# mhaseebtariq/doppel-speller

Hardware: AMD Instinct MI355X
Metric: candidate-pairs scored/sec (Jaccard top-k + Levenshtein), 100k x 500k titles (higher is better)
Workload: dtype f32 accumulate / f64 finalise (Jaccard), u8 + f64 ratio (Levenshtein)

## Files before the change

### doppel-speller_amd/csrc/ds_common.h

```cpp
#pragma once

#include <hip/hip_runtime.h>

#include <cstdarg>
#include <cstdint>
#include <cstdio>
#include <cstring>
#include <string>
#include <vector>

#include "doppel_amd.h"

namespace ds {

constexpr int kWideTileRows = 28672, kNarrowTileRows = 12288;
constexpr int64_t kNarrowMaxTruth = 5000000;
constexpr int kDenseThreads = 1024;
constexpr int kMaxQueryColumns = 128;
constexpr int kSignatureBits = 128;
constexpr int kSignatureWords = kSignatureBits / 32;
constexpr int kRowRecordWords = 8;
constexpr int kControlWords = 32;

inline uint32_t encode_sums8(float x)
{
    if (!(x >= 0.125f)) return 0u;
    uint32_t bits;
    memcpy(&bits, &x, sizeof(bits));
    const int exponent = static_cast<int>(bits >> 23) - 124;
    if (exponent > 15) return 0xfeu;
    return std::min<uint32_t>(0xfeu, (static_cast<uint32_t>(exponent) << 4) | ((bits >> 19) & 0xfu));
}

inline uint64_t mix64(uint64_t x)
{
    x ^= x >> 30;
    x *= 0xbf58476d1ce4e5b9ull;
    x ^= x >> 27;
    x *= 0x94d049bb133111ebull;
    x ^= x >> 31;
    return x;
}

enum QueryStatus : int32_t { kQueryDone = 0, kQuerySlow = 1, kQueryErrorTopN = 2, kQueryErrorArg = 3, kQueryErrorTies = 4, kQuerySlowFew = 5 };

void set_error(const char *format, ...);
void duplicate_ranks(const int64_t *rowptr, const int32_t *truth_idx, const float *sums32, int64_t V, int64_t N,
                     uint16_t *rank_out);
int hip_failed(hipError_t error, const char *what, const char *file, int line);

#define DS_HIP(call)                                                          \
    do {                                                                      \
        hipError_t ds_hip_error_ = (call);                                    \
        if (ds_hip_error_ != hipSuccess) return ::ds::hip_failed(ds_hip_error_, #call, __FILE__, __LINE__); \
    } while (0)

#define DS_REQUIRE(condition, ...)            \
    do {                                      \
        if (!(condition)) {                   \
            ::ds::set_error(__VA_ARGS__);     \
            return DS_E_ARG;                  \
        }                                     \
    } while (0)

template <typename T>
struct DeviceBuffer {
    T *ptr = nullptr;
    size_t count = 0;
    int allocate(size_t n)
    {
        release();
        if (n == 0) return DS_OK;
        DS_HIP(hipMalloc(reinterpret_cast<void **>(&ptr), n * sizeof(T)));
        count = n;
        return DS_OK;
    }
    int upload(const T *host, size_t n)
    {
        int status = allocate(n);
        if (status != DS_OK) return status;
        if (n) DS_HIP(hipMemcpy(ptr, host, n * sizeof(T), hipMemcpyHostToDevice));
        return DS_OK;
    }
    void release()
    {
// ... 68 lines not shown
```

### doppel-speller_amd/csrc/ds_jaccard_impl.inc

```
#include <cfloat>
#include <type_traits>
#include <cstdlib>

#include "ds_common.h"

namespace ds {
namespace DS_GEOMETRY_NAME {

constexpr int kTile = DS_TILE_ROWS;
constexpr uint32_t kPadWord = kTile / 2;
constexpr uint32_t kPadQuad = kPadWord * 0x10001u;
__device__ __forceinline__ uint32_t posting_row(uint32_t posting) { return ((posting & 0x7fffu) << 1) | (posting >> 15); }
constexpr int kThreads = DS_THREADS;
constexpr int kWorkgroupsPerCu = DS_WGS_PER_CU;
static_assert(kTile % 4096 == 0 && kTile < 65536, "tile rows: whole scan iterations, 15-bit word indexes");
static_assert(kThreads >= 256 && kThreads % 64 == 0, "the radix histogram is cleared by threads 0..255");
constexpr int kCandidates = DS_CANDIDATES;
constexpr int kSelectSlack = 128;
constexpr int kPtrTiles = DS_PTR_TILES;

struct JaccardArgs {
    const uint32_t *col_ptr;
    const uint16_t *postings;
    const uint16_t *posting_sums;
// ... 5 lines not shown
    const int8_t *sig_column;
    const void *row_start;
    const void *row_cols;
    int32_t forward_wide_start, forward_wide_cols;
    const int64_t *q_rowptr;
    const int32_t *q_cols;
    const double *q_maxint;
    int32_t *out_rows;
    int32_t *status;
    int32_t *control;
    int32_t *slow_list;
    const int32_t *take_order;
    unsigned long long *phase;
    int64_t n_truth;
    int64_t n_columns;
    int64_t n_queries;
    int32_t n_tiles;
    int32_t k;
    int32_t sparse_quads;
    int32_t literal_only;
    int32_t rows_sorted;
    int32_t select_min;
    int32_t select_growth;
    int64_t n_quads;
    int64_t nnz;
    float sums_min;
};

enum { kCtlQueue = 0, kCtlSlowCount = 1, kCtlErrors = 2, kCtlExact = 3, kCtlSelects = 4, kCtlSlowQueue = 5,
       kCtlSparseTiles = 6, kCtlDenseTiles = 7, kCtlSkippedColumns = 8, kCtlReason = 9 ,
       kCtlRedos = 15 ,
       kCtlRefines = 16, kCtlRawEntries = 17, kCtlSurvivors = 18, kCtlRawSparse = 19,
       kCtlBytes = 28  };

constexpr int kEpochTiles = DS_EPOCH_TILES;
static_assert(kEpochTiles >= 1 && kEpochTiles <= 256 && (kEpochTiles & (kEpochTiles - 1)) == 0, "epoch: a power of two, at most 256 tiles");
constexpr bool kEpochInBytes = static_cast<long long>(kTile + 2) * kEpochTiles > 65536;
constexpr int kEpochShift = kEpochInBytes ? 16 : 14;
static_assert(kEpochInBytes || kTile + 2 <= (1 << kEpochShift), "a local row (or a padding row, kTile + 1) and the epoch bits share 16 bits");
constexpr int kScoreWords = kTile / 2 + 16;
constexpr int kOffLo = kScoreWords * 4;
constexpr int kOffRow = kOffLo + kCandidates * 4;
constexpr int kOffRaw = kOffRow + kCandidates * 4;
constexpr int kOffRawTile = kOffRaw + (kThreads / 64) * 64 * 4;
constexpr int kOffCols = kOffRawTile + (kEpochInBytes ? (kThreads / 64) * 64 : 0);
constexpr int kOffIdf = kOffCols + kMaxQueryColumns * 4;
constexpr int kOffMass = kOffIdf + kMaxQueryColumns * 4;
constexpr int kOffBitIdf = kOffMass + kMaxQueryColumns * 4;
constexpr int kOffFixed = kOffBitIdf + kSignatureBits * 4;
constexpr int kOffRank = kOffFixed + kMaxQueryColumns * 4;
constexpr int kOffOrder = kOffRank + kMaxQueryColumns;
constexpr int kOffSigBit = kOffOrder + kMaxQueryColumns;
constexpr int kOffMassTable = kOffSigBit + kMaxQueryColumns;
constexpr int kOffPtr = kOffMassTable + 256 * 6;
constexpr int kOffHist = kOffMassTable;
constexpr int kOffQuadPrefix = kOffPtr + kMaxQueryColumns * (kPtrTiles + 1) * 4;
constexpr int kOffQuadBase = kOffQuadPrefix + kMaxQueryColumns * 4;
constexpr int kDirItems = 64, kDirColumns = 64;
constexpr int kOffDirEntry = kOffQuadBase + kMaxQueryColumns * 4;
constexpr int kOffDirMask = kOffDirEntry + 2 * kDirColumns * 8;
constexpr int kOffDirCount = kOffDirMask + 2 * kDirItems * 8;
constexpr int kOffCtrl = kOffDirCount + 2 * kDirItems;
constexpr int kFastLdsBytes = kOffCtrl + 192;
static_assert((kFastLdsBytes + 256) * kWorkgroupsPerCu <= 160 * 1024, "LDS budget of one CU exceeded");
constexpr int kExactRows = kCandidates * 24 + kMaxQueryColumns * 5 + kThreads * 2 <= kTile * 2 ? kCandidates : ((kTile * 2 - kMaxQueryColumns * 5 - kThreads * 2) / 24) & ~7;
constexpr int kExactValueOffset = kExactRows * 16;
constexpr int kExactSortedOffset = kExactValueOffset + kExactRows * 8;
constexpr int kExactCountOffset = kExactSortedOffset + kMaxQueryColumns * 5;
static_assert(kExactValueOffset % 8 == 0 && kExactCountOffset % 4 == 0 && kExactCountOffset + kThreads * 2 <= kTile * 2,
              "exact-stage scratch fits the tile");
static_assert(kMaxQueryColumns == 128, "two ballots cover the query's columns");
constexpr int kKeep = (kCandidates + kThreads - 1) / kThreads;
constexpr int kSelectTrigger = kCandidates - kSelectSlack;
constexpr int kWaves = kThreads / 64;
constexpr float kFixedOne = 65000.f;
constexpr int kProbeMaxK = kThreads / 4;
static_assert(2 * kThreads <= kCandidates - kSelectSlack, "two samples per thread fit the candidate buffer");

enum { kLQuery = 0, kLCount, kLOverflow, kLDigit, kLRemain, kLCoef, kLPre, kLCut, kLKth0, kLKth1, kLBad, kLItems,
       kLUnused12 , kLNonEssential, kLMass, kLSparse, kLSigMask , kLQuant = kLSigMask + 4 , kLEnd,
       kLStartTile = 29 ,
       kLFloor = 37 ,
       kLAhead = 38 ,
       kLTileMask = 32 , kLTileSkip = 36 ,
       kLStats = 24 ,
       kLBytes = 30  };
static_assert(kLEnd <= kLStats && kLStats + 5 <= kLBytes && kLBytes + 2 <= 32 && kLBytes % 2 == 0, "LDS control words");
static_assert(kLTileSkip < kLFloor && kLFloor < kLAhead && kLAhead + 2 <= 48, "LDS control words 32..47");

__device__ __forceinline__ int uniform(int v) { return __builtin_amdgcn_readfirstlane(v); }
__device__ __forceinline__ uint32_t uniform(uint32_t v) { return static_cast<uint32_t>(__builtin_amdgcn_readfirstlane(static_cast<int>(v))); }
__device__ __forceinline__ float uniform(float v) { return __int_as_float(__builtin_amdgcn_readfirstlane(__float_as_int(v))); }
__device__ __forceinline__ bool uniform(bool v) { return __builtin_amdgcn_readfirstlane(v ? 1 : 0) != 0; }

__device__ __forceinline__ float round_down_positive(double x)
{
    float f = static_cast<float>(x);
    if (static_cast<double>(f) > x) f = __uint_as_float(__float_as_uint(f) - 1u);
    return f;
}

__device__ __forceinline__ float round_up_positive(double x)
{
    float f = static_cast<float>(x);
    if (static_cast<double>(f) < x) f = __uint_as_float(__float_as_uint(f) + 1u);
    return f;
}
// ... 49 lines not shown
            const uint32_t key = keys[i];
            if ((key & mask) == prefix) atomicAdd(&hist[(key >> shift) & 255u], 1u);
        }
        __syncthreads();
        if (tid < 64) {
            const int b0 = 255 - 4 * lane;
            const uint32_t c0 = hist[b0], c1 = hist[b0 - 1], c2 = hist[b0 - 2], c3 = hist[b0 - 3];
            const uint32_t local = c0 + c1 + c2 + c3;
            const uint32_t inclusive = wave_inclusive_scan(local, lane);
            const uint32_t exclusive = inclusive - local;
            const uint32_t want = static_cast<uint32_t>(remaining);
            if (want > exclusive && want <= inclusive) {
                uint32_t r = want - exclusive;
                int digit = b0;
                if (r > c0) { r -= c0; digit = b0 - 1;
                    if (r > c1) { r -= c1; digit = b0 - 2;
                        if (r > c2) { r -= c2; digit = b0 - 3; } } }
                ctrl[kLDigit] = digit;
                ctrl[kLRemain] = static_cast<int32_t>(r);
            }
        }
        __syncthreads();
        prefix |= static_cast<uint32_t>(uniform(static_cast<int>(ctrl[kLDigit]))) << shift;
        mask |= 255u << shift;
        remaining = uniform(static_cast<int>(ctrl[kLRemain]));
    }
    return prefix;
}

struct Bounds {
    float coef;
    float pre;
    float mass;
    float maxint32;
};

__device__ __forceinline__ uint32_t max_of_packed8(uint4 v)
{
    typedef unsigned short packed2 __attribute__((ext_vector_type(2)));
    const packed2 a = __builtin_elementwise_max(__builtin_bit_cast(packed2, v.x), __builtin_bit_cast(packed2, v.y));
    const packed2 b = __builtin_elementwise_max(__builtin_bit_cast(packed2, v.z), __builtin_bit_cast(packed2, v.w));
    const uint32_t m = __builtin_bit_cast(uint32_t, __builtin_elementwise_max(a, b));
    return max(m & 0xffffu, m >> 16);
}

__device__ __forceinline__ uint32_t max_of_packed4(const uint32_t (&v)[4])
{
    typedef unsigned short packed2 __attribute__((ext_vector_type(2)));
    const packed2 a = __builtin_elementwise_max(__builtin_bit_cast(packed2, v[0]), __builtin_bit_cast(packed2, v[1]));
    const packed2 b = __builtin_elementwise_max(__builtin_bit_cast(packed2, v[2]), __builtin_bit_cast(packed2, v[3]));
    return __builtin_bit_cast(uint32_t, __builtin_elementwise_max(a, b));
}

__device__ __forceinline__ float decode_sums8(uint32_t code)
{
    return code == 0u ? 0.f : __uint_as_float((((code >> 4) + 124u) << 23) | ((code & 0xfu) << 19));
}

__device__ __forceinline__ bool may_qualify(float s, float sums, const Bounds &b)
{
    return s + b.mass >= b.coef * (sums + b.maxint32);
}

__device__ __forceinline__ bool candidate_key(float s, float sums, const Bounds &b, uint32_t &key)
{
    if (!(s >= b.coef * (sums + b.maxint32))) return false;
    const float denominator = sums + (b.maxint32 - s);
    const float approx = s / denominator;
    key = (denominator > 0.f && approx == approx) ? __float_as_uint(approx) : 0x7f800000u;
    return true;
}

struct Skipped {
    int count;
    uint32_t sig_mask[kSignatureWords];
};

__device__ __forceinline__ float complete_score(float s, uint4 signature, const Skipped &skipped, const float *bit_idf)
{
    const uint32_t words[kSignatureWords] = {signature.x, signature.y, signature.z, signature.w};
#pragma unroll
    for (int w = 0; w < kSignatureWords; ++w) {
        uint32_t bits = words[w] & skipped.sig_mask[w];
        while (bits) {
            s += bit_idf[w * 32 + __ffs(bits) - 1];
            bits &= bits - 1u;
        }
    }
    return s;
}


__device__ __forceinline__ void append_candidate(bool pass, uint32_t key, int32_t row, uint32_t *cand_key,
                                                 int32_t *cand_row, ControlWords ctrl, int lane)
{
    const unsigned long long votes = __ballot(pass);
    if (votes == 0) return;
    const int leader = __ffsll(votes) - 1;
    int base = 0;
    if (lane == leader) base = atomicAdd(ctrl.at(kLCount), __popcll(votes));
    base = __shfl(base, leader);
    if (pass) {
        const int slot = base + __popcll(votes & ((1ull << lane) - 1ull));
        if (slot < kCandidates) {
            cand_key[slot] = key;
            cand_row[slot] = row;
        } else {
            ctrl[kLOverflow] = 1;
        }
    }
}
// ... 8 lines not shown
    }
}
__device__ __forceinline__ bool in_bounds(int32_t *control, int site, int64_t index, int64_t limit)
{
    if (index >= 0 && index < limit) return true;
    record_violation(control, site, index, limit);
    return false;
}
#define DS_OK_INDEX(site, index, limit) in_bounds(a.control, site, static_cast<int64_t>(index), static_cast<int64_t>(limit))
#else
#define DS_OK_INDEX(site, index, limit) true
#endif

#ifdef DS_DIAGNOSTICS
#define DS_STAMP(slot)                                                     \
    do {                                                                   \
        if (a.phase != nullptr && tid == 0) {                              \
            const unsigned long long now_ = __builtin_amdgcn_s_memtime();  \
            phase_lds[slot] += now_ - stamp_;                              \
            stamp_ = now_;                                                 \
        }                                                                  \
    } while (0)
#define DS_COUNT(slot, value)                                              \
    do {                                                                   \
        if (a.phase != nullptr && tid == 0) atomicAdd(&a.control[slot], value); \
    } while (0)
#else
#define DS_STAMP(slot) do { } while (0)
#define DS_COUNT(slot, value) do { } while (0)
#endif

template <bool kCountBytes, bool kSecondSample>
__global__ __launch_bounds__(kThreads, kWorkgroupsPerCu * kThreads / 256) void ds_jaccard_topk_kernel(const void *arguments)
{
    const __attribute__((address_space(4))) JaccardArgs &a =
        *reinterpret_cast<const __attribute__((address_space(4))) JaccardArgs *>(reinterpret_cast<uintptr_t>(arguments));
#ifdef DS_DIAGNOSTICS
    unsigned long long stamp_ = a.phase != nullptr ? __builtin_amdgcn_s_memtime() : 0ull;
    __shared__ unsigned long long phase_lds[16];
    if (threadIdx.x < 16) phase_lds[threadIdx.x] = 0ull;
#endif
    extern __shared__ __align__(16) unsigned char lds[];
    uint32_t *cand_key = reinterpret_cast<uint32_t *>(lds + kOffLo);
    int32_t *cand_row = reinterpret_cast<int32_t *>(lds + kOffRow);
    int32_t *cols = reinterpret_cast<int32_t *>(lds + kOffCols);
    float *idf = reinterpret_cast<float *>(lds + kOffIdf);
    uint8_t *rank = reinterpret_cast<uint8_t *>(lds + kOffRank);
    uint8_t *order = reinterpret_cast<uint8_t *>(lds + kOffOrder);
    float *mass_upto = reinterpret_cast<float *>(lds + kOffMass);
    int8_t *sig_bit = reinterpret_cast<int8_t *>(lds + kOffSigBit);
    float *bit_idf = reinterpret_cast<float *>(lds + kOffBitIdf);
    uint32_t *fixed = reinterpret_cast<uint32_t *>(lds + kOffFixed);
    uint32_t *iscores = reinterpret_cast<uint32_t *>(lds);
    uint32_t *need32 = reinterpret_cast<uint32_t *>(lds + kOffMassTable);
    uint16_t *mass16 = reinterpret_cast<uint16_t *>(lds + kOffMassTable + 256 * 4);
    uint32_t *ptr_cache = reinterpret_cast<uint32_t *>(lds + kOffPtr);
    uint32_t *quad_prefix = reinterpret_cast<uint32_t *>(lds + kOffQuadPrefix);
    uint32_t *quad_base = reinterpret_cast<uint32_t *>(lds + kOffQuadBase);
    uint2 *dir_entry = reinterpret_cast<uint2 *>(lds + kOffDirEntry);
    uint32_t *dir_mask = reinterpret_cast<uint32_t *>(lds + kOffDirMask);
    uint8_t *dir_count = reinterpret_cast<uint8_t *>(lds + kOffDirCount);
    uint32_t *hist = reinterpret_cast<uint32_t *>(lds + kOffHist);
    const ControlWords ctrl{reinterpret_cast<int32_t *>(lds + kOffCtrl)};

    const int tid = threadIdx.x, lane = tid & 63;
    const int wave = uniform(tid >> 6);
    const int k = a.k;
    const int64_t ptr_stride = static_cast<int64_t>(a.n_tiles) + 1;
    typedef const unsigned long long __attribute__((address_space(1))) *GlobalQuads;
    auto load_quad = [](GlobalQuads base, uint32_t at) {
        const unsigned long long bits = base[at];
        return make_uint2(static_cast<uint32_t>(bits), static_cast<uint32_t>(bits >> 32));
    };
    auto own_registers = [](const void *pointer) {
        const uint64_t bits = reinterpret_cast<uint64_t>(pointer);
        const uint32_t lo = uniform(static_cast<uint32_t>(bits)), hi = uniform(static_cast<uint32_t>(bits >> 32));
        return reinterpret_cast<GlobalQuads>((static_cast<uint64_t>(hi) << 32) | lo);
    };
    const GlobalQuads quads = own_registers(a.postings), sums_quads = own_registers(a.posting_sums);
    typedef const float __attribute__((address_space(4))) *ConstantFloats;
    const ConstantFloats tile_sums_min = reinterpret_cast<ConstantFloats>(reinterpret_cast<uintptr_t>(a.tile_sums_min));
    const ConstantFloats tile_sums_max = reinterpret_cast<ConstantFloats>(reinterpret_cast<uintptr_t>(a.tile_sums_max));

    for (int i = tid * 4; i < kScoreWords; i += kThreads * 4)
        *reinterpret_cast<uint4 *>(&iscores[i]) = make_uint4(0u, 0u, 0u, 0u);
    if (tid < 5) ctrl[kLStats + tid] = 0;
    if (tid < 2) ctrl[kLBytes + tid] = 0;
    __syncthreads();
    unsigned long long *requested = reinterpret_cast<unsigned long long *>(lds + kOffCtrl + kLBytes * 4);
    uint32_t query_units = 0;
    auto count_units = [&](uint32_t units) { if constexpr (kCountBytes) query_units += units; };

    for (;;) {
        if (tid == 0) {
            ctrl[kLQuery] = atomicAdd(&a.control[kCtlQueue], 1);
            ctrl[kLCount] = 0;
            ctrl[kLOverflow] = 0;
            ctrl[kLBad] = 0;
            ctrl[kLQuant] = 0;
            ctrl[kLStartTile] = 0;
            ctrl[kLFloor] = 0;
        }
        __syncthreads();
        const int64_t position = uniform(static_cast<int>(ctrl[kLQuery]));
        if (position >= a.n_queries) break;
        const int64_t q = a.take_order != nullptr ? static_cast<int64_t>(a.take_order[position]) : position;

        const int64_t qbase = a.q_rowptr[q];
// ... 156 lines not shown
            }
            raw_count += count;
        };

        int sparse_retries = 0;
        uint32_t dir_copy = 0;
        constexpr int kRound = 3;
        bool ahead = false;
        uint2 quad[kRound], quad_info[kRound];
        uint32_t quad_value[kRound];
        bool live[kRound];
#pragma unroll
        for (int u = 0; u < kRound; ++u) {
            quad[u] = quad_info[u] = make_uint2(0u, 0u);
            quad_value[u] = 0u;
            live[u] = false;
        }
        const int span = n > 0 ? min(a.n_tiles, max(kPtrTiles, kMaxQueryColumns * (kPtrTiles + 1) / n - 1)) : kPtrTiles;
        int block_start = 0, block_end = 0;
        const bool sorted = a.rows_sorted != 0;
        const int start_tile = sorted ? min(uniform(static_cast<int>(ctrl[kLStartTile])), a.n_tiles - 1) : 0;
        int epoch_start = start_tile, epoch_last = start_tile;
        int down_next = start_tile - 1;
        int up_next = start_tile + 1;
        bool descending = false;
        int run_left = 0;
        int b = start_tile;
        while (!slow) {
            bool redo_tile = false;
            const float tile_min = tile_sums_min[b];
            if (__builtin_expect(b < block_start || b >= block_end, 0)) {
                block_start = descending ? max(0, min(b, epoch_last - span + 1)) : b;
                block_end = block_start + span;
                __syncthreads();
                const int width = min(span, a.n_tiles - block_start) + 1;
                for (int e = tid; e < n * (span + 1); e += kThreads) {
                    const int j = e / (span + 1), i = e - j * (span + 1);
                    ptr_cache[e] = (i < width && DS_OK_INDEX(2, static_cast<int64_t>(cols[j]) * ptr_stride + block_start + i,
                                                            a.n_columns * ptr_stride))
                                       ? a.col_ptr[static_cast<int64_t>(cols[j]) * ptr_stride + block_start + i]
                                       : 0u;
                }
                count_units(static_cast<uint32_t>(n * width + 1) >> 1);
                __syncthreads();
            }
            const int bt = b - block_start;
            bounds.mass = pending_mass;
            if (__builtin_expect(rebuild_mass_table, 0)) {
                rebuild_mass_table = false;
                tables_fresh = true;
                if (tid < 4) ctrl[kLTileMask + tid] = static_cast<int32_t>(ctrl[kLSigMask + tid]);
                if (tid == 4) ctrl[kLTileSkip] = non_essential;
                if (tid < 256) {
                    const uint32_t skipped8 = static_cast<uint32_t>(ctrl[kLSigMask]) & 0xffu;
                    float rest = bounds.mass, some = 0.f;
                    for (int g = 0; g < 8; ++g) {
                        if (!((skipped8 >> g) & 1u)) continue;
                        rest -= bit_idf[g];
                        if ((tid >> g) & 1) some += bit_idf[g];
                    }
                    if (rest < 0.f) rest = 0.f;
                    const float value = (rest + some) * (1.f + 3.814697265625e-06f) + 1e-30f;
                    const float mass = value < bounds.mass ? value : bounds.mass;
                    const float mass_units = mass * to_fixed_high + 2.5f;
                    mass16[tid] = static_cast<uint16_t>(mass_units < 65535.f ? mass_units : 65535.f);
                    const float need_units = bounds.coef * (decode_sums8(tid) + maxint32) * to_fixed_low - 2.5f;
                    need32[tid] = tid == 255 ? 0x7fffffffu
                                             : static_cast<uint32_t>(need_units < 0.f ? 0.f : (need_units < 65535.f ? need_units : 65535.f));
                }
            }
            const bool sparse = tight && sparse_mode;
            auto build_map = [&](int tile_bt, uint32_t copy, bool at_start, bool &directory) {
                uint32_t *const mask = dir_mask + copy * (2 * kDirItems);
                if (!at_start) {
                    mask[lane] = 0u;
                    mask[64 + lane] = 0u;
                }
                uint2 *const entry = dir_entry + copy * kDirColumns;
                uint8_t *const count = dir_count + copy * kDirItems;
                uint32_t quads_of[2] = {0u, 0u}, begin_of[2] = {0u, 0u};
#pragma unroll
                for (int h = 0; h < 2; ++h) {
                    const int j = lane + 64 * h;
                    if (j < n && rank[j] >= non_essential) {
                        begin_of[h] = ptr_cache[j * (span + 1) + tile_bt];
                        quads_of[h] = ptr_cache[j * (span + 1) + tile_bt + 1] - begin_of[h];
                    }
                }
                const uint32_t scan0 = wave_inclusive_scan(quads_of[0], lane);
                uint32_t total = static_cast<uint32_t>(__builtin_amdgcn_readlane(static_cast<int>(scan0), 63));
                const uint32_t before0 = scan0 - quads_of[0];
                uint32_t before1 = 0;
                const unsigned long long started0 = __ballot(quads_of[0] != 0u);
                unsigned long long started1 = 0ull;
                if (n > 64) {
                    const uint32_t scan1 = wave_inclusive_scan(quads_of[1], lane);
                    before1 = total + scan1 - quads_of[1];
                    total += static_cast<uint32_t>(__builtin_amdgcn_readlane(static_cast<int>(scan1), 63));
                    started1 = __ballot(quads_of[1] != 0u);
                }
                const int lists0 = __popcll(started0), lists = lists0 + __popcll(started1);
                directory = total <= static_cast<uint32_t>(kDirItems * 64) && lists <= kDirColumns;
                if (directory) {
                    const uint32_t below0 = __builtin_amdgcn_mbcnt_hi(static_cast<uint32_t>(started0 >> 32),
                                                                      __builtin_amdgcn_mbcnt_lo(static_cast<uint32_t>(started0), 0u));
                    if (quads_of[0] != 0u) {
                        entry[below0] = make_uint2(begin_of[0] - before0, fixed[lane]);
                        atomicOr(&mask[(before0 >> 6) * 2 + ((before0 >> 5) & 1u)], 1u << (before0 & 31u));
                    }
                    if (n > 64) {
                        const uint32_t below1 = lists0 + __builtin_amdgcn_mbcnt_hi(static_cast<uint32_t>(started1 >> 32),
                                                                                   __builtin_amdgcn_mbcnt_lo(static_cast<uint32_t>(started1), 0u));
                        if (quads_of[1] != 0u) {
                            entry[below1] = make_uint2(begin_of[1] - before1, fixed[lane + 64]);
                            atomicOr(&mask[(before1 >> 6) * 2 + ((before1 >> 5) & 1u)], 1u << (before1 & 31u));
                        }
                    }
                    const uint2 bits = *reinterpret_cast<const uint2 *>(&mask[2 * lane]);
                    const uint32_t starts = static_cast<uint32_t>(__popc(bits.x) + __popc(bits.y));
                    count[lane] = static_cast<uint8_t>(wave_inclusive_scan(starts, lane) - starts);
                } else if (at_start) {
                    quad_prefix[lane] = lane < n ? before0 : 0xffffffffu;
                    quad_base[lane] = begin_of[0] - before0;
                    if (n > 64) {
                        quad_prefix[lane + 64] = lane + 64 < n ? before1 : 0xffffffffu;
                        quad_base[lane + 64] = begin_of[1] - before1;
                    }
                }
                return total;
            };
            auto locate_in = [&](uint32_t copy, bool directory, uint32_t total, int at, uint32_t &first, uint32_t &value) {
                const uint32_t g = static_cast<uint32_t>(at) * 64u + lane;
                if (directory) {
                    const uint2 bits = *reinterpret_cast<const uint2 *>(&dir_mask[copy * (2 * kDirItems) + 2 * at]);
                    const uint32_t before = dir_count[copy * kDirItems + at];
                    const uint32_t below = __builtin_amdgcn_mbcnt_hi(bits.y, __builtin_amdgcn_mbcnt_lo(bits.x, 0u));
                    const uint32_t own = ((lane < 32 ? bits.x : bits.y) >> (lane & 31)) & 1u;
                    const uint2 entry = dir_entry[copy * kDirColumns + ((before + below + own - 1u) & (kDirColumns - 1))];
                    first = entry.x + g;
                    value = entry.y;
                } else {
                    uint32_t c = 0;
#pragma unroll
                    for (uint32_t bit = kMaxQueryColumns / 2; bit > 0; bit >>= 1) {
                        const uint32_t t = c + bit;
                        c = quad_prefix[t] <= g ? t : c;
                    }
                    first = quad_base[c] + g;
                    value = fixed[c];
                }
                return g < total;
            };
            auto request_round = [&](uint32_t copy, bool directory, uint32_t total, int items, int round, bool keep,
                                     bool count_sparse, uint2 (&q)[kRound], uint2 (&info)[kRound], uint32_t (&value)[kRound],
                                     bool (&alive)[kRound]) {
#pragma unroll
                for (int u = 0; u < kRound; ++u) {
                    const int at = wave + (round + u) * kWaves;
                    uint32_t first = 0;
                    value[u] = 0;
                    alive[u] = at < items && locate_in(copy, directory, total, at, first, value[u]) &&
                               DS_OK_INDEX(3, first, a.n_quads);
                    q[u] = alive[u] ? load_quad(quads, first) : make_uint2(kPadQuad, kPadQuad);
                    if (keep)
                        info[u] = alive[u] ? load_quad(sums_quads, first) : make_uint2(0xff00ff00u, 0xff00ff00u);
                    if constexpr (kCountBytes) {
                        const unsigned long long loaded = __ballot(alive[u]);
                        if (count_sparse && lane == 0)
                            atomicAdd(requested, static_cast<unsigned long long>(__popcll(loaded)) * (keep ? 16u : 8u));
                    }
                }
            };
            raw_tile_base = static_cast<int64_t>(epoch_start) * kTile;
            raw_epoch_bits = kEpochInBytes ? static_cast<uint32_t>(b - epoch_start)
                                           : static_cast<uint32_t>(b - epoch_start) << (kEpochShift & 15);
            const bool epoch_end = b >= epoch_last;
            const bool map_ahead = !epoch_end && b + 1 < block_end;
            const uint32_t tile_copy = dir_copy;
            if (!map_ahead) {
                uint32_t *const other = dir_mask + (tile_copy ^ 1u) * (2 * kDirItems);
                other[lane] = 0u;
                other[64 + lane] = 0u;
            }
            bool use_directory = false;
            uint32_t total_quads = 0;
            if (ahead) {
                const uint32_t built = uniform(static_cast<uint32_t>(ctrl[kLAhead + static_cast<int>(tile_copy)]));
                total_quads = built & 0x7fffffffu;
                use_directory = (built >> 31) != 0u;
#ifdef DS_BOUNDS_CHECK
                {
                    uint32_t mine = 0;
                    for (int j = lane; j < n; j += 64)
                        if (rank[j] >= non_essential) mine += ptr_cache[j * (span + 1) + bt + 1] - ptr_cache[j * (span + 1) + bt];
                    for (int d = 32; d > 0; d >>= 1) mine += __shfl_xor(mine, d);
                    if (mine != total_quads) record_violation(a.control, 11, static_cast<int64_t>(total_quads), static_cast<int64_t>(mine));
                }
#endif
            }
            if (!use_directory) total_quads = build_map(bt, tile_copy, true, use_directory);
            ahead = map_ahead;
            dir_copy ^= 1u;
            const int n_items = static_cast<int>((total_quads + 63u) >> 6);
            auto locate = [&](int at, uint32_t &first, uint32_t &value) {
                return locate_in(tile_copy, use_directory, total_quads, at, first, value);
            };
            if constexpr (kCountBytes) {
                if (!sparse) count_units(total_quads);
            }
            DS_STAMP(1);

            const int64_t tile_base = static_cast<int64_t>(b) * kTile;
            int count_at_step = sparse ? 0 : uniform(static_cast<int>(ctrl[kLCount]));
            Bounds here = bounds;
            auto passes = [&](float s, float sums_lower_bound, float row_mass) {
                return (s > 0.f) & (s + row_mass >= here.pre) &
                       (s + row_mass >= here.coef * (sums_lower_bound + here.maxint32));
            };
// ... 3 lines not shown
#pragma unroll
                for (int e = 0; e < 4; ++e)
                    pass[e] = passes(static_cast<float>(fixed_score[e]) * from_fixed, sums_lower_bound[e], row_mass[e]);
                if (__ballot(pass[0] || pass[1] || pass[2] || pass[3]) == 0) return;
#pragma unroll
                for (int e = 0; e < 4; ++e) append_raw(pass[e], fixed_score[e], local[e]);
            };

            int kept_round = 0;
#pragma unroll
            for (int u = 0; u < kRound; ++u) live[u] = false;
            const int count_before = count_at_step;
            for (int round = 0; wave + round * kWaves < n_items; round += kRound) {
                const bool keep = sparse && wave + (round + kRound) * kWaves >= n_items;
                kept_round = round;
                request_round(tile_copy, use_directory, total_quads, n_items, round, keep, sparse, quad, quad_info, quad_value, live);
                if (map_ahead && round == 0 && wave == (b & (kWaves - 1))) {
                    bool directory;
                    const uint32_t total = build_map(bt + 1, tile_copy ^ 1u, false, directory);
                    if (lane == 0) {
                        ctrl[kLAhead + static_cast<int>(tile_copy ^ 1u)] = static_cast<int32_t>(total | (directory ? 0x80000000u : 0u));
                    }
                }
                if (sparse) DS_STAMP(10);
#pragma unroll
                for (int u = 0; u < kRound; ++u) {
                    if (!live[u]) continue;
                    const uint32_t shifted = quad_value[u] << ((quad[u].x >> 11) & 16u);
                    atomicAdd(&iscores[quad[u].x & 0x7fffu], shifted);
                    atomicAdd(&iscores[(quad[u].x >> 16) & 0x7fffu], shifted);
                    atomicAdd(&iscores[quad[u].y & 0x7fffu], shifted);
                    atomicAdd(&iscores[(quad[u].y >> 16) & 0x7fffu], shifted);
                }
            }
            if (map_ahead && wave >= n_items && wave == (b & (kWaves - 1))) {
                bool directory;
                const uint32_t total = build_map(bt + 1, tile_copy ^ 1u, false, directory);
                if (lane == 0) {
                    ctrl[kLAhead + static_cast<int>(tile_copy ^ 1u)] = static_cast<int32_t>(total | (directory ? 0x80000000u : 0u));
                }
            }
            if (sparse) DS_STAMP(15);
            __syncthreads();
            DS_STAMP(sparse ? 6 : 2);
            {
                const float gate = uniform(bounds.coef * (tile_min + maxint32) * (1.f - 3.814697265625e-06f));
                if (gate > here.pre) here.pre = gate;
            }

            if (sparse) {
                ++sparse_tiles;
                if (__builtin_expect(tables_fresh, 0)) {
                    tables_fresh = false;
                    mass_units_max = uniform(static_cast<uint32_t>(mass16[255]));
                }
                const uint32_t gate_fixed = [&]() {
                    const float units = here.pre * to_fixed_low - 2.f;
                    const uint32_t gate = units > 0.f ? static_cast<uint32_t>(units) : 0u;
                    return max(gate, mass_units_max);
                }();
                auto collect = [&]() {
#pragma unroll
                    for (int u = 0; u < kRound; ++u) {
                        if (__ballot(live[u]) == 0) continue;
                        const uint32_t word[4] = {quad[u].x & 0x7fffu, (quad[u].x >> 16) & 0x7fffu, quad[u].y & 0x7fffu,
                                                  (quad[u].y >> 16) & 0x7fffu};
                        const uint32_t shift = (quad[u].x >> 11) & 16u;
                        const uint32_t info[4] = {quad_info[u].x & 0xffffu, quad_info[u].x >> 16, quad_info[u].y & 0xffffu,
                                                  quad_info[u].y >> 16};
                        uint32_t least[4];
                        uint32_t taken[4];
                        uint32_t before[4];
#pragma unroll
                        for (int e = 0; e < 4; ++e) before[e] = 0u;
                        if (live[u]) {
#pragma unroll
                            for (int e = 0; e < 4; ++e)
                                before[e] = atomicAnd(&iscores[word[e]], ~(0xffffu << shift));
                        }
#pragma unroll
                        for (int e = 0; e < 4; ++e) taken[e] = (before[e] >> shift) & 0xffffu;
#ifdef DS_DIAGNOSTICS
                        if (a.phase != nullptr) {
                            int touched = 0, level1 = 0;
                            for (int e = 0; e < 4; ++e) {
                                touched += taken[e] != 0u;
                                level1 += taken[e] != 0u && taken[e] + mass16[255] >= gate_fixed;
                            }
                            for (int d = 32; d > 0; d >>= 1) { touched += __shfl_xor(touched, d); level1 += __shfl_xor(level1, d); }
                            if (lane == 0) { atomicAdd(&a.control[20], touched); atomicAdd(&a.control[21], level1);
                                             atomicAdd(&a.control[22], 1); atomicAdd(&a.control[23], level1 != 0); }
                        }
#endif
                        if (__ballot(((max_of_packed4(before) >> shift) & 0xffffu) >= gate_fixed - mass_units_max) == 0) continue;
#pragma unroll
                        for (int e = 0; e < 4; ++e)
                            least[e] = max(gate_fixed, need32[info[e] >> 8]) - mass16[info[e] & 0xffu];
                        bool pass[4];
#pragma unroll
                        for (int e = 0; e < 4; ++e)
                            pass[e] = taken[e] >= least[e];
                        if (__ballot(pass[0] | pass[1] | pass[2] | pass[3]) == 0) continue;
#pragma unroll
                        for (int e = 0; e < 4; ++e) append_raw(pass[e], taken[e], (word[e] << 1) | (shift >> 4));
                    }
                };
                collect();
                for (int round = 0; round < kept_round; round += kRound) {
#pragma unroll
                    for (int u = 0; u < kRound; ++u) {
                        const int at = wave + (round + u) * kWaves;
                        uint32_t first = 0, value = 0;
                        live[u] = at < n_items && locate(at, first, value) && DS_OK_INDEX(3, first, a.n_quads);
                        quad[u] = live[u] ? load_quad(quads, first) : make_uint2(kPadQuad, kPadQuad);
                        quad_info[u] = live[u] ? load_quad(sums_quads, first) : make_uint2(0xff00ff00u, 0xff00ff00u);
                        if constexpr (kCountBytes) {
                            const unsigned long long loaded = __ballot(live[u]);
                            if (lane == 0) atomicAdd(requested, static_cast<unsigned long long>(__popcll(loaded)) * 16u);
                        }
                    }
                    collect();
                }
                DS_STAMP(13);
                if (epoch_end) flush_raw();
                DS_STAMP(14);
                __syncthreads();
                DS_STAMP(7);
                if (__builtin_expect(uniform(static_cast<int>(ctrl[kLOverflow])) != 0, 0)) {
                    if (++sparse_retries > 5) { slow = true; reason = 2; break; }
                    wanted_in = uniform(static_cast<int>(ctrl[kLCount]));
                    floor_shift = min(sparse_retries - 1, 3);
                    __syncthreads();
                    if (tid == 0) {
                        ctrl[kLCount] = kCandidates;
                        ctrl[kLOverflow] = 0;
                        atomicAdd(&a.control[kCtlRedos], 1);
                    }
                    if (tid < 2 * kDirItems) dir_mask[dir_copy * (2 * kDirItems) + tid] = 0u;
                    ahead = false;
                    __syncthreads();
                    redo_tile = true;
                    raw_count = 0;
                } else {
                    if (epoch_end) sparse_retries = 0;
                    DS_COUNT(kCtlRawSparse, ctrl[kLCount] - count_before);
                    if (!epoch_end) {
                        ++b;
                        continue;
                    }
                }
            }

            const int64_t rows_left = a.n_truth - tile_base;
            const int limit = rows_left >= kTile ? kTile : static_cast<int>((rows_left + 7) & ~int64_t(7));
            int r0 = sparse ? limit : 0;
            if (!sparse) ++dense_tiles;
            bool select_now = sparse && (redo_tile || (epoch_end && uniform(static_cast<int>(ctrl[kLCount])) >= next_select));
            int retries = 0;
            bool probed = false;
            int32_t drop_lo = redo_tile ? static_cast<int32_t>(raw_tile_base) : 0;
            int32_t drop_hi = redo_tile ? static_cast<int32_t>(tile_base + kTile) : 0;
            bool force_pending = redo_tile;
            while (r0 < limit || select_now) {
                bool force_select = force_pending;
                force_pending = false;
                if (r0 < limit && !tight && !probed && k <= (kSecondSample ? 2 : 1) * kProbeMaxK && count_at_step == 0) {
                    probed = true;
                    const float tile_max = tile_sums_max[b];
// ... 76 lines not shown
                        }
                    }
                    flush_raw();
                    __syncthreads();
                    DS_STAMP(3);
                    last_appended = uniform(static_cast<int>(ctrl[kLCount])) - count_at_step;
                    if (uniform(static_cast<int>(ctrl[kLOverflow]))) {
                        if (!recoverable || ++retries > 6) { slow = true; reason = 3; break; }
                        wanted_in = uniform(static_cast<int>(ctrl[kLCount]));
                        floor_shift = min(retries - 1, 3);
                        __syncthreads();
                        if (tid == 0) {
                            ctrl[kLCount] = kCandidates;
                            ctrl[kLOverflow] = 0;
                        }
                        __syncthreads();
                        force_select = true;
                        drop_lo = static_cast<int32_t>(tile_base + r0);
                        drop_hi = static_cast<int32_t>(tile_base + r1);
                    } else {
                        if (recoverable) {
                            for (int idx = r0 + tid * 8; idx < r1; idx += kThreads * 8)
                                *reinterpret_cast<uint4 *>(&iscores[idx >> 1]) = make_uint4(0u, 0u, 0u, 0u);
                            __syncthreads();
                            DS_STAMP(9);
                        }
                        r0 = r1;
                        retries = 0;
                    }
                    DS_STAMP(12);
                }
                select_now = false;
                const int m = uniform(static_cast<int>(ctrl[kLCount]));
                if ((m < next_select && !force_select) || m < k) {
                    if (force_select) { slow = true; reason = 3; break; }
                    continue;
                }
                const uint32_t tau_key = radix_select_kth(cand_key, m, k, hist, ctrl, 2);
                ++selects;
                if (wanted_in > 0) {
                    const int rank = static_cast<int>(static_cast<long long>(max((kSelectTrigger - 64) >> floor_shift, k + 16)) * m / max(wanted_in, m));
                    wanted_in = 0;
                    const uint32_t pivot = radix_select_kth(cand_key, m, max(1, min(m, rank)), hist, ctrl, 4);
                    if (tid == 0 && static_cast<uint32_t>(ctrl[kLFloor]) < pivot) ctrl[kLFloor] = static_cast<int32_t>(pivot);
                }
                if (wave == 0) {
                    const double tau = static_cast<double>(__uint_as_float(tau_key));
                    const double cut_value = tau - 2.0 * error_margin() - 2e-6;
                    float new_coef = 0.f, new_pre = FLT_MIN, new_cut = 0.f;
                    if (tau_key < 0x7f800000u && cut_value > 0.0) {
                        const double c = cut_value / (1.0 + cut_value) * (1.0 - 9.5367431640625e-07);
                        new_coef = round_down_positive(c);
                        new_cut = round_down_positive(cut_value);
                        const double p = static_cast<double>(new_coef) *
                                         (static_cast<double>(a.sums_min) + static_cast<double>(maxint32)) *
                                         (1.0 - 9.5367431640625e-07);
                        new_pre = p > static_cast<double>(FLT_MIN) ? round_down_positive(p) : FLT_MIN;
                    }
                    int skip_count = 0;
                    {
                        const bool ok0 = lane < n && mass_upto[lane] < new_pre && sig_bit[order[lane]] >= 0;
                        const bool ok1 = lane + 64 < n && mass_upto[lane + 64] < new_pre && sig_bit[order[lane + 64]] >= 0;
                        const unsigned long long v0 = __ballot(ok0), v1 = __ballot(ok1);
                        skip_count = ~v0 ? __ffsll(static_cast<long long>(~v0)) - 1
                                         : 64 + (~v1 ? __ffsll(static_cast<long long>(~v1)) - 1 : 64);
                    }
                    uint32_t mask_bits[kSignatureWords] = {0u, 0u, 0u, 0u};
#pragma unroll
                    for (int h = 0; h < 2; ++h) {
                        const int r = lane + 64 * h;
                        if (r < skip_count) {
                            const int bit = sig_bit[order[r]];
#pragma unroll
                            for (int w = 0; w < kSignatureWords; ++w)
                                if ((bit >> 5) == w) mask_bits[w] |= 1u << (bit & 31);
                        }
                    }
#pragma unroll
                    for (int w = 0; w < kSignatureWords; ++w)
                        for (int d = 32; d > 0; d >>= 1) mask_bits[w] |= __shfl_xor(mask_bits[w], d);
                    uint32_t essential_quads = 0;
                    count_units(static_cast<uint32_t>(n));
#pragma unroll
                    for (int h = 0; h < 2; ++h) {
                        const int j = lane + 64 * h;
                        if (j < n && rank[j] >= skip_count)
                            essential_quads += a.col_ptr[static_cast<int64_t>(cols[j]) * ptr_stride + a.n_tiles] -
                                               a.col_ptr[static_cast<int64_t>(cols[j]) * ptr_stride];
                    }
                    for (int d = 32; d > 0; d >>= 1) essential_quads += __shfl_xor(essential_quads, d);
                    if (lane == 0) {
                        ctrl[kLSparse] = essential_quads / static_cast<uint32_t>(a.n_tiles) <=
                                         static_cast<uint32_t>(a.sparse_quads);
                        for (int w = 0; w < kSignatureWords; ++w) ctrl[kLSigMask + w] = static_cast<int32_t>(mask_bits[w]);
                        ctrl[kLCoef] = __float_as_int(new_coef);
                        ctrl[kLPre] = __float_as_int(new_pre);
                        ctrl[kLCut] = __float_as_int(new_cut);
                        ctrl[kLNonEssential] = skip_count;
                        ctrl[kLMass] = __float_as_int(skip_count > 0 ? mass_upto[skip_count - 1] : 0.f);
                    }
                }
                __syncthreads();
                bounds.coef = uniform(__int_as_float(ctrl[kLCoef]));
                bounds.pre = uniform(__int_as_float(ctrl[kLPre]));
                here.coef = bounds.coef;
                {
                    const float gate = uniform(bounds.coef * (tile_min + maxint32) * (1.f - 3.814697265625e-06f));
                    here.pre = gate > bounds.pre ? gate : bounds.pre;
// ... 1060 lines not shown
```

### doppel-speller_amd/csrc/ds_runtime.hip

```cpp
#include <algorithm>
#include <chrono>
#include <cstdlib>
#include <cstring>

#include "ds_common.h"
#include "ds_host.h"

namespace ds {

static thread_local std::string g_last_error;

void set_error(const char *format, ...)
{
    char buffer[1024];
    va_list args;
    va_start(args, format);
    vsnprintf(buffer, sizeof(buffer), format, args);
    va_end(args);
    g_last_error = buffer;
}

int hip_failed(hipError_t error, const char *what, const char *file, int line)
{
    set_error("HIP error %d (%s) at %s:%d in %s", static_cast<int>(error), hipGetErrorString(error), file, line, what);
// ... 344 lines not shown
        const size_t top = static_cast<size_t>(std::min<int64_t>(V, ds::kSignatureBits));
        std::partial_sort(by_length.begin(), by_length.begin() + top, by_length.end(), [&](int64_t x, int64_t y) {
            const int64_t lx = rowptr[x + 1] - rowptr[x], ly = rowptr[y + 1] - rowptr[y];
            return lx != ly ? lx > ly : x < y;
        });
        for (size_t bit = 0; bit < top; ++bit) {
            const int64_t g = by_length[bit];
            if ((rowptr[g + 1] - rowptr[g]) * 256 < N) break;
            sig_column[static_cast<size_t>(g)] = static_cast<int8_t>(bit);
        }
    }
    bool literal_only = false;
    for (int64_t g = 0; g < V && !literal_only; ++g) literal_only = !(idf32[g] >= 0.f && idf32[g] < 1e30f);
    std::vector<uint32_t> records(static_cast<size_t>(N) * ds::kRowRecordWords, 0u);
    {
        std::vector<double> row_total(static_cast<size_t>(N), 0.0);
        ds::for_postings_by_row_range(rowptr, truth_idx, V, N, threads, [&](int, int64_t g, int64_t from, int64_t to) {
            const double value = idf32[g];
            for (int64_t p = from; p < to; ++p) row_total[static_cast<size_t>(truth_idx[p])] += value;
            const int bit = sig_column[static_cast<size_t>(g)];
            if (bit >= 0)
                for (int64_t p = from; p < to; ++p)
                    records[static_cast<size_t>(truth_idx[p]) * ds::kRowRecordWords + static_cast<size_t>(bit >> 5)] |= 1u << (bit & 31);
        });
        std::vector<uint8_t> violated(static_cast<size_t>(threads), 0);
        ds::parallel_ranges(N, threads, [&](int thread, int64_t begin, int64_t end) {
            bool bad = false;
            for (int64_t t = begin; t < end && !bad; ++t)
                bad = !(sums32[t] >= 0.f && sums32[t] < 1e30f) ||
                      static_cast<double>(sums32[t]) < row_total[static_cast<size_t>(t)] * (1.0 - 1e-4);
            violated[static_cast<size_t>(thread)] = bad;
        });
        for (uint8_t bad : violated) literal_only = literal_only || bad;
    }
    phase("signatures + row totals");

    const uint16_t pad_word = static_cast<uint16_t>(tile_rows / 2);
    std::vector<uint16_t> postings(static_cast<size_t>(quads) * 4), posting_sums(static_cast<size_t>(quads) * 4);
    ds::parallel_dynamic(V, 32, threads, [&](int, int64_t column_begin, int64_t column_end) {
        for (int64_t g = column_begin; g < column_end; ++g) {
            const uint32_t *row = col_ptr.data() + g * stride;
            int64_t p = rowptr[g];
            while (p < rowptr[g + 1]) {
                const int64_t b = truth_idx[p] / tile_rows, tile_first = b * tile_rows, tile_end = tile_first + tile_rows;
                int64_t last = p, even = 0;
                for (; last < rowptr[g + 1] && truth_idx[last] < tile_end; ++last) even += ((truth_idx[last] - tile_first) & 1) == 0;
                uint64_t write[2] = {static_cast<uint64_t>(row[b]) * 4u,
                                     (static_cast<uint64_t>(row[b]) + static_cast<uint64_t>(even + 3) / 4u) * 4u};
                const uint64_t part_end[2] = {write[1], static_cast<uint64_t>(row[b + 1]) * 4u};
                for (; p < last; ++p) {
                    const int64_t t = truth_idx[p];
                    const uint32_t local = static_cast<uint32_t>(t - tile_first);
                    uint64_t &at = write[local & 1u];
                    posting_sums[at] = static_cast<uint16_t>((ds::encode_sums8(sums32[t]) << 8) |
                                                              (records[static_cast<size_t>(t) * ds::kRowRecordWords] & 0xffu));
                    postings[at++] = static_cast<uint16_t>(((local & 1u) << 15) | (local >> 1));
                }
                for (int part = 0; part < 2; ++part)
                    for (uint64_t i = write[part]; i < part_end[part]; ++i) {
                        postings[i] = static_cast<uint16_t>((part << 15) | pad_word);
                        posting_sums[i] = static_cast<uint16_t>(0xff00);
                    }
            }
        }
    });
    phase("postings");
    std::vector<uint16_t> dup_rank(static_cast<size_t>(N), 0u);
    ds::duplicate_ranks(rowptr, truth_idx, sums32, V, N, dup_rank.data());
    phase("duplicate ranks");
    ds::parallel_ranges(N, threads, [&](int, int64_t begin, int64_t end) {
        for (int64_t t = begin; t < end; ++t) {
            uint32_t *record = records.data() + static_cast<size_t>(t) * ds::kRowRecordWords;
            std::memcpy(&record[4], &sums32[t], sizeof(float));
            record[5] = dup_rank[static_cast<size_t>(t)];
            record[6] = static_cast<uint32_t>(original[static_cast<size_t>(t)]);
        }
    });
    const bool wide_start = nnz >= (int64_t(1) << 32) - 1, wide_cols = V > 65536;
    std::vector<int64_t> row_start(static_cast<size_t>(N) + 1, 0);
    ds::for_postings_by_row_range(rowptr, truth_idx, V, N, threads, [&](int, int64_t, int64_t from, int64_t to) {
        for (int64_t p = from; p < to; ++p) ++row_start[static_cast<size_t>(truth_idx[p]) + 1];
    });
    for (int64_t t = 0; t < N; ++t) row_start[static_cast<size_t>(t) + 1] += row_start[static_cast<size_t>(t)];
    {
        if (wide_cols) image.row_cols32.resize(static_cast<size_t>(nnz)); else image.row_cols16.resize(static_cast<size_t>(nnz));
        int32_t *const cols32 = image.row_cols32.data();
        uint16_t *const cols16 = image.row_cols16.data();
        std::vector<int64_t> fill(row_start.begin(), row_start.end() - 1);
        ds::for_postings_by_row_range(rowptr, truth_idx, V, N, threads, [&](int, int64_t g, int64_t from, int64_t to) {
            if (wide_cols)
                for (int64_t p = from; p < to; ++p) cols32[fill[static_cast<size_t>(truth_idx[p])]++] = static_cast<int32_t>(g);
            else
                for (int64_t p = from; p < to; ++p) cols16[fill[static_cast<size_t>(truth_idx[p])]++] = static_cast<uint16_t>(g);
        });
    }
    if (wide_start) {
        image.row_start64.swap(row_start);
    } else {
        image.row_start32.resize(row_start.size());
        for (size_t t = 0; t < row_start.size(); ++t) image.row_start32[t] = static_cast<uint32_t>(row_start[t]);
    }
    image.wide_start = wide_start;
    image.wide_cols = wide_cols;
    phase("forward index");
    image.n_tiles = n_tiles;
    image.tile_rows = tile_rows;
    image.nnz = nnz;
    image.quads = quads;
    image.sums_min = sums_min;
    image.literal_only = literal_only;
    image.rows_sorted = sort_rows;
    image.col_ptr.swap(col_ptr);
    image.records.swap(records);
    image.postings.swap(postings);
// ... 280 lines not shown
```

Baseline: 66.23 million.

## Replace per-posting sums8 gate with 16-bit signature mass bounds

Per-posting metadata now stores 16 signature bits instead of an 8-bit encoded row-sum plus 8 signature bits. The pruning bound becomes a full-mass minus a low-byte missing-mass table plus a high-byte table, and padding postings are excluded explicitly via the pad word check. The precomputed threshold also uses a band edge derived from the cut to tighten the minimum sums. The goal is tighter candidate pruning from more signature bits, traded against dropping the per-row sums constraint, which may admit more candidates.

```diff
diff --git a/doppel-speller_amd/csrc/ds_common.h b/doppel-speller_amd/csrc/ds_common.h
--- a/doppel-speller_amd/csrc/ds_common.h
+++ b/doppel-speller_amd/csrc/ds_common.h
@@ -21,16 +21,6 @@
 constexpr int kSignatureWords = kSignatureBits / 32;
 constexpr int kRowRecordWords = 8;
 constexpr int kControlWords = 32;
-
-inline uint32_t encode_sums8(float x)
-{
-    if (!(x >= 0.125f)) return 0u;
-    uint32_t bits;
-    memcpy(&bits, &x, sizeof(bits));
-    const int exponent = static_cast<int>(bits >> 23) - 124;
-    if (exponent > 15) return 0xfeu;
-    return std::min<uint32_t>(0xfeu, (static_cast<uint32_t>(exponent) << 4) | ((bits >> 19) & 0xfu));
-}
 
 inline uint64_t mix64(uint64_t x)
 {
diff --git a/doppel-speller_amd/csrc/ds_jaccard_impl.inc b/doppel-speller_amd/csrc/ds_jaccard_impl.inc
--- a/doppel-speller_amd/csrc/ds_jaccard_impl.inc
+++ b/doppel-speller_amd/csrc/ds_jaccard_impl.inc
@@ -81,7 +81,7 @@
 constexpr int kOffOrder = kOffRank + kMaxQueryColumns;
 constexpr int kOffSigBit = kOffOrder + kMaxQueryColumns;
 constexpr int kOffMassTable = kOffSigBit + kMaxQueryColumns;
-constexpr int kOffPtr = kOffMassTable + 256 * 6;
+constexpr int kOffPtr = kOffMassTable + 256 * 4;
 constexpr int kOffHist = kOffMassTable;
 constexpr int kOffQuadPrefix = kOffPtr + kMaxQueryColumns * (kPtrTiles + 1) * 4;
 constexpr int kOffQuadBase = kOffQuadPrefix + kMaxQueryColumns * 4;
@@ -237,11 +237,6 @@
     return __builtin_bit_cast(uint32_t, __builtin_elementwise_max(a, b));
 }
 
-__device__ __forceinline__ float decode_sums8(uint32_t code)
-{
-    return code == 0u ? 0.f : __uint_as_float((((code >> 4) + 124u) << 23) | ((code & 0xfu) << 19));
-}
-
 __device__ __forceinline__ bool may_qualify(float s, float sums, const Bounds &b)
 {
     return s + b.mass >= b.coef * (sums + b.maxint32);
@@ -356,8 +351,8 @@
     float *bit_idf = reinterpret_cast<float *>(lds + kOffBitIdf);
     uint32_t *fixed = reinterpret_cast<uint32_t *>(lds + kOffFixed);
     uint32_t *iscores = reinterpret_cast<uint32_t *>(lds);
-    uint32_t *need32 = reinterpret_cast<uint32_t *>(lds + kOffMassTable);
-    uint16_t *mass16 = reinterpret_cast<uint16_t *>(lds + kOffMassTable + 256 * 4);
+    uint16_t *mass_low = reinterpret_cast<uint16_t *>(lds + kOffMassTable);
+    uint16_t *mass_high = mass_low + 256;
     uint32_t *ptr_cache = reinterpret_cast<uint32_t *>(lds + kOffPtr);
     uint32_t *quad_prefix = reinterpret_cast<uint32_t *>(lds + kOffQuadPrefix);
     uint32_t *quad_base = reinterpret_cast<uint32_t *>(lds + kOffQuadBase);
@@ -620,21 +615,18 @@
                 if (tid < 4) ctrl[kLTileMask + tid] = static_cast<int32_t>(ctrl[kLSigMask + tid]);
                 if (tid == 4) ctrl[kLTileSkip] = non_essential;
                 if (tid < 256) {
-                    const uint32_t skipped8 = static_cast<uint32_t>(ctrl[kLSigMask]) & 0xffu;
-                    float rest = bounds.mass, some = 0.f;
+                    const uint32_t skipped16 = static_cast<uint32_t>(ctrl[kLSigMask]) & 0xffffu;
+                    float lacks_low = 0.f, lacks_high = 0.f;
                     for (int g = 0; g < 8; ++g) {
-                        if (!((skipped8 >> g) & 1u)) continue;
-                        rest -= bit_idf[g];
-                        if ((tid >> g) & 1) some += bit_idf[g];
-                    }
-                    if (rest < 0.f) rest = 0.f;
-                    const float value = (rest + some) * (1.f + 3.814697265625e-06f) + 1e-30f;
-                    const float mass = value < bounds.mass ? value : bounds.mass;
-                    const float mass_units = mass * to_fixed_high + 2.5f;
-                    mass16[tid] = static_cast<uint16_t>(mass_units < 65535.f ? mass_units : 65535.f);
-                    const float need_units = bounds.coef * (decode_sums8(tid) + maxint32) * to_fixed_low - 2.5f;
-                    need32[tid] = tid == 255 ? 0x7fffffffu
-                                             : static_cast<uint32_t>(need_units < 0.f ? 0.f : (need_units < 65535.f ? need_units : 65535.f));
+                        if (((skipped16 >> g) & 1u) && !((tid >> g) & 1)) lacks_low += bit_idf[g];
+                        if (((skipped16 >> (g + 8)) & 1u) && !((tid >> g) & 1)) lacks_high += bit_idf[g + 8];
+                    }
+                    const float full_units = bounds.mass * to_fixed_high + 2.5f;
+                    const uint32_t full = static_cast<uint32_t>(full_units < 65535.f ? full_units : 65535.f);
+                    const uint32_t low = static_cast<uint32_t>(lacks_low * (1.f - 3.814697265625e-06f) * to_fixed_low);
+                    const uint32_t high = static_cast<uint32_t>(lacks_high * (1.f - 3.814697265625e-06f) * to_fixed_low);
+                    mass_low[tid] = static_cast<uint16_t>(full - min(low, full));
+                    mass_high[tid] = static_cast<uint16_t>(min(high, 65535u));
                 }
             }
             const bool sparse = tight && sparse_mode;
@@ -731,7 +723,7 @@
                                DS_OK_INDEX(3, first, a.n_quads);
                     q[u] = alive[u] ? load_quad(quads, first) : make_uint2(kPadQuad, kPadQuad);
                     if (keep)
-                        info[u] = alive[u] ? load_quad(sums_quads, first) : make_uint2(0xff00ff00u, 0xff00ff00u);
+                        info[u] = alive[u] ? load_quad(sums_quads, first) : make_uint2(0u, 0u);
                     if constexpr (kCountBytes) {
                         const unsigned long long loaded = __ballot(alive[u]);
                         if (count_sparse && lane == 0)
@@ -841,7 +833,7 @@
                 ++sparse_tiles;
                 if (__builtin_expect(tables_fresh, 0)) {
                     tables_fresh = false;
-                    mass_units_max = uniform(static_cast<uint32_t>(mass16[255]));
+                    mass_units_max = uniform(static_cast<uint32_t>(mass_low[255]));
                 }
                 const uint32_t gate_fixed = [&]() {
                     const float units = here.pre * to_fixed_low - 2.f;
@@ -874,7 +866,7 @@
                             int touched = 0, level1 = 0;
                             for (int e = 0; e < 4; ++e) {
                                 touched += taken[e] != 0u;
-                                level1 += taken[e] != 0u && taken[e] + mass16[255] >= gate_fixed;
+                                level1 += taken[e] != 0u && taken[e] + mass_units_max >= gate_fixed;
                             }
                             for (int d = 32; d > 0; d >>= 1) { touched += __shfl_xor(touched, d); level1 += __shfl_xor(level1, d); }
                             if (lane == 0) { atomicAdd(&a.control[20], touched); atomicAdd(&a.control[21], level1);
@@ -884,11 +876,11 @@
                         if (__ballot(((max_of_packed4(before) >> shift) & 0xffffu) >= gate_fixed - mass_units_max) == 0) continue;
 #pragma unroll
                         for (int e = 0; e < 4; ++e)
-                            least[e] = max(gate_fixed, need32[info[e] >> 8]) - mass16[info[e] & 0xffu];
+                            least[e] = gate_fixed - mass_low[info[e] & 0xffu] + mass_high[info[e] >> 8];
                         bool pass[4];
 #pragma unroll
                         for (int e = 0; e < 4; ++e)
-                            pass[e] = taken[e] >= least[e];
+                            pass[e] = (taken[e] >= least[e]) & (word[e] != kPadWord);
                         if (__ballot(pass[0] | pass[1] | pass[2] | pass[3]) == 0) continue;
 #pragma unroll
                         for (int e = 0; e < 4; ++e) append_raw(pass[e], taken[e], (word[e] << 1) | (shift >> 4));
@@ -902,7 +894,7 @@
                         uint32_t first = 0, value = 0;
                         live[u] = at < n_items && locate(at, first, value) && DS_OK_INDEX(3, first, a.n_quads);
                         quad[u] = live[u] ? load_quad(quads, first) : make_uint2(kPadQuad, kPadQuad);
-                        quad_info[u] = live[u] ? load_quad(sums_quads, first) : make_uint2(0xff00ff00u, 0xff00ff00u);
+                        quad_info[u] = live[u] ? load_quad(sums_quads, first) : make_uint2(0u, 0u);
                         if constexpr (kCountBytes) {
                             const unsigned long long loaded = __ballot(live[u]);
                             if (lane == 0) atomicAdd(requested, static_cast<unsigned long long>(__popcll(loaded)) * 16u);
@@ -1085,8 +1077,10 @@
                         const double c = cut_value / (1.0 + cut_value) * (1.0 - 9.5367431640625e-07);
                         new_coef = round_down_positive(c);
                         new_cut = round_down_positive(cut_value);
-                        const double p = static_cast<double>(new_coef) *
-                                         (static_cast<double>(a.sums_min) + static_cast<double>(maxint32)) *
+                        const double band_edge = static_cast<double>(new_cut) * static_cast<double>(maxint32) * (1.0 - 1e-5);
+                        const double sums_floor = band_edge > static_cast<double>(a.sums_min) ? band_edge
+                                                                                              : static_cast<double>(a.sums_min);
+                        const double p = static_cast<double>(new_coef) * (sums_floor + static_cast<double>(maxint32)) *
                                          (1.0 - 9.5367431640625e-07);
                         new_pre = p > static_cast<double>(FLT_MIN) ? round_down_positive(p) : FLT_MIN;
                     }
diff --git a/doppel-speller_amd/csrc/ds_runtime.hip b/doppel-speller_amd/csrc/ds_runtime.hip
--- a/doppel-speller_amd/csrc/ds_runtime.hip
+++ b/doppel-speller_amd/csrc/ds_runtime.hip
@@ -420,14 +420,13 @@
                     const int64_t t = truth_idx[p];
                     const uint32_t local = static_cast<uint32_t>(t - tile_first);
                     uint64_t &at = write[local & 1u];
-                    posting_sums[at] = static_cast<uint16_t>((ds::encode_sums8(sums32[t]) << 8) |
-                                                              (records[static_cast<size_t>(t) * ds::kRowRecordWords] & 0xffu));
+                    posting_sums[at] = static_cast<uint16_t>(records[static_cast<size_t>(t) * ds::kRowRecordWords] & 0xffffu);
                     postings[at++] = static_cast<uint16_t>(((local & 1u) << 15) | (local >> 1));
                 }
                 for (int part = 0; part < 2; ++part)
                     for (uint64_t i = write[part]; i < part_end[part]; ++i) {
                         postings[i] = static_cast<uint16_t>((part << 15) | pad_word);
-                        posting_sums[i] = static_cast<uint16_t>(0xff00);
+                        posting_sums[i] = static_cast<uint16_t>(0);
                     }
             }
         }
```

Result: faster. 67.27 million, median of 6 (+1.6%).
